# AHupuJR/REFID

Measured on AMD Instinct MI355X. Metric: interpolated frames/sec (train step) GoPro 256x256 11+1, higher is better.
Workload: dtype f32

## Files before the change

refid_amd/csrc/common.h:

```cpp
#pragma once
#include <hip/hip_runtime.h>
#include <stdint.h>
#include <stdio.h>
#include <stdarg.h>
#include <atomic>
#include "../../include/refid_hip.h"

typedef float f32x4 __attribute__((ext_vector_type(4)));
typedef float f32x16 __attribute__((ext_vector_type(16)));

void refid_set_error(const char* fmt, ...);

#define REFID_CHECK(cond, ...)                    \
    do {                                          \
        if (!(cond)) {                            \
            refid_set_error(__VA_ARGS__);         \
            return 1;                             \
        }                                         \
    } while (0)

#define REFID_LAUNCH_CHECK(what)                                                   \
    do {                                                                           \
        hipError_t e__ = hipGetLastError();                                        \
        if (e__ != hipSuccess) {                                                   \
// ... 8 lines not shown
#pragma unroll
        for (int k = 0; k < 4; ++k) v[k] = lrelu(v[k], slope);
        asm volatile("" ::: "memory");
    }
}

template <int LPP>
__device__ __forceinline__ float refid_wave_rows_sum(float v) {
#pragma unroll
    for (int o = LPP; o < 64; o <<= 1) v += __shfl_xor(v, o, 64);
    return v;
}

int refid_launch_sum_rows_f64(const double* part, int rows, int n, double* out, hipStream_t st);

static inline int cdiv(int a, int b) { return (a + b - 1) / b; }
static inline int round_up(int a, int b) { return cdiv(a, b) * b; }

template <class K>
static inline int refid_lds_attr_once(std::atomic<unsigned long long>& done, K kernel, int bytes, const char* what) {
    int dev = 0;
    if (hipGetDevice(&dev) != hipSuccess || dev < 0 || dev > 63) { refid_set_error("%s: hipGetDevice failed", what); return 2; }
    if ((done.load(std::memory_order_relaxed) >> dev) & 1ull) return 0;
    hipError_t e = hipFuncSetAttribute(reinterpret_cast<const void*>(kernel), hipFuncAttributeMaxDynamicSharedMemorySize, bytes);
    if (e != hipSuccess) { refid_set_error("%s: LDS attribute: %s", what, hipGetErrorString(e)); return 2; }
    done.fetch_or(1ull << dev, std::memory_order_relaxed);
    return 0;
}
```

refid_amd/csrc/conv_args.h:

```cpp
#pragma once

struct ConvKArgs {
    const float* inA; const float* inB;
    int ldA, ldB, Ca, Ctot;
    const float* w; const float* bias;
    float* out; int ldO;
    const float* res; int ldR;
    const float* mask; int ldM;
    int N, H, W, Ho, Wo;
    int Cout, CoutPad, coBase;
    int pad, nchunks, tilesX, tilesY;
    float slopePre, slopePost, slopeMask;
    long long wClsStride;
    int vecOK;
    int ncot;
    int bf16;
    int ksplit = 1;
    long long wsStride = 0;
    int gridTiles = 0;
    const float* add2 = nullptr; float* out2 = nullptr; int ldA2 = 0, ldO2 = 0;
    int maskMode = 0;
    int shuffle = 0;
    int patchW = 0, patchRow = 0;
};


size_t refid_wino3x3_workspace_bytes(const ConvKArgs& a, int split_mode);
int refid_launch_wino3x3(const ConvKArgs& a, float* ws, size_t ws_bytes, int split_mode, int tile_hint, hipStream_t st);
int refid_launch_splitk_finish(const ConvKArgs& f, const float* ws, int ldW, long long npix, hipStream_t st);
bool refid_wino6_eligible(const ConvKArgs& a);
size_t refid_wino6_workspace_bytes(const ConvKArgs& a, int split_mode);
int refid_launch_wino6(const ConvKArgs& a, float* ws, size_t ws_bytes, int split_mode, int tile_hint, int terms, hipStream_t st);
bool refid_split3x3_eligible(const ConvKArgs& a);
int refid_launch_split3x3(const ConvKArgs& a, int terms, int mode, int cus, int split_mode, hipStream_t st);
struct PwExtra {
    const float* lnG = nullptr; const float* lnB = nullptr; float lnEps = 0.f; float* lnOut = nullptr; int ldLn = 0;
    const float* pool = nullptr; int poolParts = 0; float invHW = 0.f; int hw = 0; int seC = 0;
    const float* seW1 = nullptr; const float* seB1 = nullptr; const float* seW2 = nullptr; const float* seB2 = nullptr;
// ... 7 lines not shown
```

refid_amd/csrc/conv_split.hip:

```cpp
#include "common.h"
#include "conv_args.h"

#ifndef REFID_SPLIT_ABLATE
#define REFID_SPLIT_ABLATE 0
#endif

namespace {

typedef __bf16 bf16x8 __attribute__((ext_vector_type(8)));
typedef _Float16 f16x8 __attribute__((ext_vector_type(8)));
typedef _Float16 f16x2 __attribute__((ext_vector_type(2)));
typedef float f32x2 __attribute__((ext_vector_type(2)));
constexpr int F16_TGT = 8;
constexpr int F16_SLACK = 6;
constexpr int F16_E0 = F16_TGT + 1;
constexpr int F16_HEADER = 64;
constexpr int TW = 32;
constexpr int KC = 8;
constexpr int NTH = 256;
constexpr int OOB = -1;
__device__ __forceinline__ int cdiv_dev(int a, int b) { return (a + b - 1) / b; }

#ifdef REFID_SPLIT_TRACE
__device__ unsigned long long* g_split_trace = nullptr;
// ... 57 lines not shown
__device__ __forceinline__ void split8h(const f32x4& v0, const f32x4& v1, f32x4 (&pl)[2]) {
    f16x8 h, l;
#pragma unroll
    for (int k = 0; k < 8; k += 2) {
        const f32x2 ab = {k < 4 ? v0[k] : v1[k - 4], k < 4 ? v0[k + 1] : v1[k - 3]};
        const f16x2 hh = __builtin_convertvector(ab, f16x2);
        const f32x2 r = ab - __builtin_convertvector(hh, f32x2);
        const f16x2 ll = __builtin_convertvector(r, f16x2);
        h[k] = hh[0]; h[k + 1] = hh[1];
        l[k] = ll[0]; l[k + 1] = ll[1];
    }
    pl[0] = __builtin_bit_cast(f32x4, h);
    pl[1] = __builtin_bit_cast(f32x4, l);
}

template <int MT, int NT, int PL, int KS, int MODE, bool F16 = false>
__global__ __launch_bounds__(NTH, 2) void conv_split_kernel(const ConvKArgs a) {
    using C = SCfg<MT, NT, PL, KS, MODE, F16>;
    static_assert(!F16 || PL == 2, "the fp16 form has two planes");
    constexpr int HP = C::HP, BN = C::BN, HWD = C::HWD, NTAP = C::NTAP, NSTEP = C::NSTEP;
    static_assert(MODE != 1 || KS == 2, "MODE 1: a stage = the two column positions of a block");
    extern __shared__ __attribute__((aligned(16))) char smem[];
    f32x4* sA = reinterpret_cast<f32x4*>(smem);
    f32x4* sB = sA + KS * PL * C::A_SLOTS;
    float* sM = reinterpret_cast<float*>(sB + KS * PL * C::B_SLOTS);

    const int tid = threadIdx.x;
    const int lane = tid & 63, wave = tid >> 6;
    const int li = lane & 31, kh = lane >> 5;

    const int xcd = blockIdx.x & 7, slot = blockIdx.x >> 3;
// ... 81 lines not shown
                    if constexpr (MODE == 1) vo = sub == 0 ? (sy1 ? voB[it] : voA[it]) : (sy1 ? vo1x[1][it] : vo1x[0][it]);
                    else vo = fromA ? voA[it] : voB[it];
                    if (!cok) vo = OOB;
                    ra[sub][it][i & 1] = __builtin_bit_cast(f32x4, __builtin_amdgcn_raw_buffer_load_b128(rs, vo, soff + 16 * (i & 1), 0));
                } else {
                    const int it = i - 2 * C::A_ITEMS;
                    int vo = voW[it];
                    if constexpr (MODE == 2) vo |= (ch * KS + sub < nsub) ? 0 : OOB;
                    rb[sub][it] = __builtin_bit_cast(
                        f32x4, __builtin_amdgcn_raw_buffer_load_b128(rsW, vo, (ch * KS + sub) * wChunk, 0));
                }
            }
        }
    };
    auto load_chunk = [&](int ch) { load_part(ch, -1); };
    auto post_max = [&]() {
        float tm = 0.f;
#pragma unroll
        for (int sub = 0; sub < KS; ++sub)
#pragma unroll
            for (int it = 0; it < C::A_ITEMS; ++it)
#pragma unroll
                for (int h = 0; h < 2; ++h) {
                    const f32x4 v = ra[sub][it][h];
                    tm = fmaxf(fmaxf(tm, fmaxf(fabsf(v[0]), fabsf(v[1]))), fmaxf(fabsf(v[2]), fabsf(v[3])));
                }
#pragma unroll
        for (int o = 32; o >= 1; o >>= 1) tm = fmaxf(tm, __shfl_xor(tm, o));
        if (lane == 0) sM[wave] = tm;
    };
// ... 60 lines not shown
            const int dy = (j == 0) ? 1 : (py ? 2 : 0);
            const int dx = (kh == 0) ? 1 : (px ? 2 : 0);
            aoff[j] = (wave * MT + dy) * HWD + dx + li;
        }
    }
    const f32x4* pB = sB + kh * BN + li;

    load_chunk(0);
    if constexpr (F16) {
        post_max();
        __syncthreads();
        store_chunk(stage_scale());
    } else {
        store_chunk();
    }
    __syncthreads();
    SPLIT_STAMP(1);

    for (int ch = 0; ch < ((REFID_SPLIT_ABLATE == 5 || REFID_SPLIT_ABLATE == 7) ? 0 : a.nchunks); ++ch) {
        const bool more = ch + 1 < a.nchunks;
        SPLIT_KSTAMP(ch, 0);
        SPLIT_KSTAMP(ch, 1);
#pragma unroll
        for (int sj = 0; sj < NSTEP * KS; ++sj) {
            const int sub = sj / NSTEP, j = sj % NSTEP;
            if (more && REFID_SPLIT_ABLATE != 4) load_part(ch + 1, sj);
            f32x4 af[PL][MT], bf[PL][NT];
#pragma unroll
            for (int p = 0; p < PL; ++p) {
#pragma unroll
                for (int m = 0; m < MT; ++m)
                    af[p][m] = REFID_SPLIT_ABLATE == 8 ? ra[0][0][m & 1] : sA[(sub * PL + p) * C::A_SLOTS + m * HWD + aoff[j]];
#pragma unroll
                for (int nn = 0; nn < NT; ++nn)
// ... 2 lines not shown
#pragma unroll
            for (int e = 0; e < (REFID_SPLIT_ABLATE == 1 ? 0 : TERMS); ++e)
#pragma unroll
                for (int m = 0; m < MT; ++m)
#pragma unroll
                    for (int nn = 0; nn < NT; ++nn) {
                        if constexpr (F16)
                            acc[m][nn] = __builtin_amdgcn_mfma_f32_32x32x16_f16(
                                __builtin_bit_cast(f16x8, bf[TB[e]][nn]), __builtin_bit_cast(f16x8, af[TA[e]][m]),
                                acc[m][nn], 0, 0, 0);
                        else
                            acc[m][nn] = __builtin_amdgcn_mfma_f32_32x32x16_bf16(
                                __builtin_bit_cast(bf16x8, bf[TB[e]][nn]), __builtin_bit_cast(bf16x8, af[TA[e]][m]),
                                acc[m][nn], 0, 0, 0);
                    }
            __builtin_amdgcn_sched_barrier(0);
        }
        SPLIT_KSTAMP(ch, 2);
        if constexpr (F16) {
            if (more) post_max();
        }
        __syncthreads();
        SPLIT_KSTAMP(ch, 3);
#ifdef REFID_SPLIT_TRACE
        __builtin_amdgcn_s_waitcnt(0x0F70);
#endif
        SPLIT_KSTAMP(ch, 4);
        if (more) {
            if constexpr (F16) store_chunk(stage_scale());
            else store_chunk();
            SPLIT_KSTAMP(ch, 5);
            __syncthreads();
        }
        SPLIT_KSTAMP(ch, 6);
    }
    SPLIT_STAMP(2);

    constexpr int C4 = C::C4, XS = C::XS;
    constexpr int EIT = (32 * C4) / 64;
    auto opix = [&](int oy, int ox) -> long long {
        if (MODE == 2) return (long long)(n * 2 * a.Ho + 2 * oy + py) * (2 * a.Wo) + 2 * ox + px;
        return (long long)(n * a.Ho + oy) * a.Wo + ox;
    };
    f32x4* ex = reinterpret_cast<f32x4*>(smem) + wave * (32 * XS);
#pragma unroll
    for (int m = 0; m < MT; ++m) {
        const int oy = oy0 + wave * MT + m;
        f32x4 pres[EIT], pmask[EIT];
        const bool pre = a.vecOK && (a.res != nullptr || a.mask != nullptr) && REFID_SPLIT_ABLATE != 6 && REFID_SPLIT_ABLATE != 7;
// ... 60 lines not shown
                for (int k = 0; k < 4; ++k) {
                    if (j0 + k >= a.Cout) break;
                    float tv = v[k];
                    if (a.res) tv += a.res[op * a.ldR + j0 + k];
                    tv = lrelu(tv, a.slopePost);
                    if (a.mask) tv *= (a.mask[op * a.ldM + j0 + k] > 0.f) ? 1.f : a.slopeMask;
                    a.out[op * a.ldO + j0 + k] = tv;
                    if (a.out2) a.out2[op * a.ldO2 + j0 + k] = tv + a.add2[op * a.ldA2 + j0 + k];
                }
            }
        }
    }
    SPLIT_STAMP(3);
}

template <int MT, int NT, int PL, int KS, int MODE, bool F16 = false>
int launch_split(const ConvKArgs& ka, hipStream_t st) {
    using C = SCfg<MT, NT, PL, KS, MODE, F16>;
    static std::atomic<unsigned long long> attr_done{0};
    if (int rc = refid_lds_attr_once(attr_done, &conv_split_kernel<MT, NT, PL, KS, MODE, F16>, C::LDS_BYTES, "conv_split")) return rc;
    ConvKArgs a = ka;
    a.tilesX = cdiv(a.Wo, TW);
    a.tilesY = cdiv(a.Ho, C::TH);
    a.nchunks = (MODE == 1) ? 2 * cdiv(a.Ctot, KC) : cdiv(a.Ctot, KC * KS);
    a.ncot = cdiv(a.Cout, C::BN);
    const int tiles = a.tilesX * a.tilesY * a.N;
    dim3 grid(cdiv(tiles, 8) * 8 * a.ncot, MODE == 2 ? 4 : 1);
    hipLaunchKernelGGL((conv_split_kernel<MT, NT, PL, KS, MODE, F16>), grid, dim3(NTH), C::LDS_BYTES, st, a);
    REFID_LAUNCH_CHECK("conv_split");
    return 0;
}

template <int PL, int MODE, bool F16 = false>
int launch_split_pl(const ConvKArgs& a, bool wide, bool tall, hipStream_t st) {
    constexpr int KS = (MODE == 0) ? 1 : 2;
    if (wide) return tall ? launch_split<2, 2, PL, KS, MODE, F16>(a, st) : launch_split<1, 2, PL, KS, MODE, F16>(a, st);
    return tall ? launch_split<2, 1, PL, KS, MODE, F16>(a, st) : launch_split<1, 1, PL, KS, MODE, F16>(a, st);
}

}

#ifdef REFID_SPLIT_TRACE
extern "C" int refid_split_trace_set(unsigned long long* wg_stamps, unsigned long long* k_stamps, int wg) {
    if (hipMemcpyToSymbol(HIP_SYMBOL(g_split_trace), &wg_stamps, sizeof(wg_stamps)) != hipSuccess) return 1;
    if (hipMemcpyToSymbol(HIP_SYMBOL(g_split_ktrace), &k_stamps, sizeof(k_stamps)) != hipSuccess) return 1;
// ... 38 lines not shown
```

refid_amd/csrc/conv_wino6.hip:

```cpp
#include "common.h"
#include "conv_args.h"
#include <algorithm>
#include <cstdlib>

#ifndef REFID_WINO6_ABLATE
#define REFID_WINO6_ABLATE 0
#endif

namespace {

constexpr int TW = 32;
constexpr int KC = 16;
constexpr int HWD = TW + 2;
constexpr int TH = 4;
constexpr int ROWP = 40;
constexpr int PLANE = 6 * ROWP + 5;
constexpr int R_F4 = 4 * PLANE;
constexpr int HP = (TH + 2) * HWD;
constexpr int R_ITEMS = (4 * HP + 255) / 256;
constexpr int lds_bytes(int nt) { return nt == 2 ? 64 * 66 * 16 : (32 * 66 * 16 > 2 * R_F4 * 16 ? 32 * 66 * 16 : 2 * R_F4 * 16); }
constexpr int OOB = -1;
typedef __bf16 bf16x8 __attribute__((ext_vector_type(8)));
typedef _Float16 f16x8 __attribute__((ext_vector_type(8)));
typedef _Float16 f16x2 __attribute__((ext_vector_type(2)));
// ... 34 lines not shown
    pl[0] = __builtin_bit_cast(f32x4, h);
    pl[1] = __builtin_bit_cast(f32x4, l);
}

__device__ __forceinline__ void round8h(const f32x4& v0, const f32x4& v1, f32x4 (&pl)[3]) {
    f16x8 h;
#pragma unroll
    for (int k = 0; k < 8; k += 2) {
        const f32x2 ab = {k < 4 ? v0[k] : v1[k - 4], k < 4 ? v0[k + 1] : v1[k - 3]};
        const f16x2 hh = __builtin_convertvector(ab, f16x2);
        h[k] = hh[0]; h[k + 1] = hh[1];
    }
    pl[0] = __builtin_bit_cast(f32x4, h);
}

template <int NT, bool F16, bool ONE = false>
__global__ __launch_bounds__(256, NT == 2 ? 2 : 3) void conv_wino6_kernel(const ConvKArgs a) {
    constexpr int BN = 32 * NT;
    static_assert(F16 || !ONE, "the one-product form is an fp16 form");
    constexpr int NPL = ONE ? 1 : (F16 ? 2 : 3);
    constexpr int NPR = ONE ? 1 : ((REFID_WINO6_ABLATE == 14 || REFID_WINO6_ABLATE == 15) ? 3 : (F16 ? 3 : 6));
    extern __shared__ __attribute__((aligned(16))) char smem[];
    f32x4* sR = reinterpret_cast<f32x4*>(smem);

    const int tid = threadIdx.x;
    const int lane = tid & 63, wave = tid >> 6;
    const int li = lane & 31, kh = lane >> 5;
    const int ti = wave;
    if (REFID_WINO6_ABLATE == 20 && a.N > 0) return;
    if (REFID_WINO6_ABLATE == 21 && a.N > 0) { __syncthreads(); if (tid == 12345) a.out[0] = 1.f; return; }

// ... 66 lines not shown
        for (int it = 0; it < R_ITEMS; ++it) sR[buf * R_F4 + sdst[it]] = src[it];
    };
    auto load_u = [&](int ch, int j, f32x4 (&dst)[NPL][NT]) {
        const bool in = ch < kc1;
        const int so = (REFID_WINO6_ABLATE == 1 ? 0 : ch) * uChunk + j * uXi;
#pragma unroll
        for (int p = 0; p < ((REFID_WINO6_ABLATE == 14 || REFID_WINO6_ABLATE == 15) && !ONE ? 2 : NPL); ++p)
#pragma unroll
            for (int nt = 0; nt < NT; ++nt) {
                if (REFID_WINO6_ABLATE == 13 && nt == 1) { dst[p][nt] = dst[p][0]; continue; }
                dst[p][nt] = __builtin_bit_cast(
                    f32x4, __builtin_amdgcn_raw_buffer_load_b128(rsW, in ? voU[nt] : OOB, in ? so + p * uPlane : 0, 0));
            }
    };

    f32x16 acc[4][NT];
#pragma unroll
    for (int j = 0; j < 4; ++j)
#pragma unroll
        for (int t = 0; t < NT; ++t)
#pragma unroll
            for (int r = 0; r < 16; ++r) acc[j][t][r] = 0.f;

    const int rowP = (ti == 0) ? 0 : ((ti == 2) ? 2 : 1);
    const int rowM = (ti == 0) ? 2 : ((ti == 1) ? 2 : ((ti == 2) ? 1 : 3));
    const float sgn = (ti == 1) ? 1.f : -1.f;
    const int tbase = 2 * kh * PLANE + (2 * (li >> 4)) * ROWP + (li & 15);
    const int offP = tbase + rowP * ROWP, offM = tbase + rowM * ROWP;
    constexpr int BOFF[4] = {0, 20, 1, 21};

    constexpr int TA[6] = {0, 0, 1, 0, 2, 1};
    constexpr int TB[6] = {0, 1, 0, 2, 0, 1};

    f32x4 uA[NPL][NT], uB[NPL][NT];
    auto phase = [&](int ch) {
        const int lc = ch - kc0;
        if (REFID_WINO6_ABLATE != 7 && REFID_WINO6_ABLATE != 8) {
            store_raw((lc + 1) & 1, rr);
            load_raw(ch + 2, rr);
#ifdef REFID_WINO6_PIN
            __builtin_amdgcn_sched_barrier(0x38F);
#endif
        }
        const f32x4* r = sR + (lc & 1) * R_F4;
        f32x4 t[2][4];
#pragma unroll
        for (int qq = 0; qq < 2; ++qq)
#pragma unroll
            for (int b = 0; b < 4; ++b) t[qq][b] = r[qq * PLANE + offP + BOFF[b]] + r[qq * PLANE + offM + BOFF[b]] * sgn;
        if constexpr (F16 && REFID_WINO6_ABLATE != 16) {
// ... 43 lines not shown
            else if (F16 && REFID_WINO6_ABLATE == 18) { pl[0] = v[0]; pl[1] = v[1]; }
            else if constexpr (ONE) round8h(v[0], v[1], pl);
            else if constexpr (F16) split8h(v[0], v[1], pl);
            else split8(v[0], v[1], pl);
#pragma unroll
            for (int e = 0; e < NPR; ++e)
#pragma unroll
                for (int nt = 0; nt < NT; ++nt) {
                    if constexpr (F16)
                        acc[j][nt] = __builtin_amdgcn_mfma_f32_32x32x16_f16(
                            __builtin_bit_cast(f16x8, cur[TB[e]][nt]), __builtin_bit_cast(f16x8, pl[TA[e]]), acc[j][nt], 0, 0, 0);
                    else
                        acc[j][nt] = __builtin_amdgcn_mfma_f32_32x32x16_bf16(
                            __builtin_bit_cast(bf16x8, cur[TB[e]][nt]), __builtin_bit_cast(bf16x8, pl[TA[e]]), acc[j][nt], 0, 0, 0);
                }
        }
        __syncthreads();
    };

    {
        f32x4 rr0[R_ITEMS];
#if REFID_WINO6_ABLATE == 19
        int keep[R_ITEMS];
#pragma unroll
        for (int it = 0; it < R_ITEMS; ++it) {
            keep[it] = pixo[it];
            const int hp = (tid >> 2) + it * 64;
            const int row = hp / HWD, col = hp % HWD;
            pixo[it] = (hp < HP && row >= a.pad && col >= a.pad) ? (row - a.pad) * a.W + (col - a.pad) : OOB;
        }
#endif
        load_raw(kc0, rr0);
        load_raw(kc0 + 1, rr);
#if REFID_WINO6_ABLATE == 19
#pragma unroll
        for (int it = 0; it < R_ITEMS; ++it) pixo[it] = keep[it];
#endif
        load_u(kc0, 0, uA);
        if (REFID_WINO6_ABLATE == 6 || REFID_WINO6_ABLATE == 8) load_u(kc0, 1, uB);
        store_raw(0, rr0);
    }
    __syncthreads();

    if (REFID_WINO6_ABLATE != 3 && REFID_WINO6_ABLATE != 10)
        for (int ch = kc0; ch < kc1; ++ch) phase(ch);

    constexpr int XL = 66;
    f32x4* xch = reinterpret_cast<f32x4*>(smem);
#pragma unroll
    for (int t = 0; t < NT; ++t)
#pragma unroll
        for (int rq = 0; rq < 4; ++rq) {
            f32x4 r0, r1;
#pragma unroll
            for (int k = 0; k < 4; ++k) {
                const int r = 4 * rq + k;
                r0[k] = acc[0][t][r] + acc[1][t][r] + acc[2][t][r];
                r1[k] = acc[1][t][r] - acc[2][t][r] - acc[3][t][r];
                if constexpr (F16) {
                    r0[k] = ldexpf(r0[k], eRef - 127 - F16_TGT - eU);
// ... 111 lines not shown
    a.nchunks = cdiv(a.Ctot, KC);
    a.ncot = cdiv(a.Cout, bn);
    p.grid = dim3(round_up(a.tilesX * a.tilesY * a.N, 8) * a.ncot);
    const int nwg = (split_mode == 2) ? (int)p.grid.x : a.tilesX * a.tilesY * a.ncot * 8;
    int ks = 1;
    if (split_mode && nwg <= 256 && a.nchunks >= 8) {
        ks = 512 / nwg;
        if (ks > a.nchunks / 4) ks = a.nchunks / 4;
        if (ks > 8) ks = 8;
        if (ks < 1) ks = 1;
    }
    p.ks = ks;
    return p;
}

template <int NT, bool F16, bool ONE = false>
int launch_wino6_t(const ConvKArgs& a, dim3 grid, hipStream_t st, const char* what) {
    static std::atomic<unsigned long long> done{0};
    if (int rc = refid_lds_attr_once(done, &conv_wino6_kernel<NT, F16, ONE>, lds_bytes(NT), "conv_wino6")) return rc;
    hipLaunchKernelGGL((conv_wino6_kernel<NT, F16, ONE>), grid, dim3(256), lds_bytes(NT), st, a);
    REFID_LAUNCH_CHECK(what);
    return 0;
}

template <int NT>
int launch_wino6(const ConvKArgs& a, int terms, dim3 grid, hipStream_t st, const char* what) {
    if (terms == 1) return launch_wino6_t<NT, true, true>(a, grid, st, what);
    return terms == 3 ? launch_wino6_t<NT, true>(a, grid, st, what) : launch_wino6_t<NT, false>(a, grid, st, what);
}

}

bool refid_wino6_eligible(const ConvKArgs& a) {
    const long long lim = 0x7fffffffLL;
    return a.Cout >= 1 && a.Ctot % 4 == 0 && (a.inB == nullptr || a.Ca % KC == 0) &&
           (long long)a.N * a.H * a.W * a.ldA * 4 < lim && (!a.inB || (long long)a.N * a.H * a.W * a.ldB * 4 < lim) &&
           (long long)cdiv(a.Ctot, KC) * 16 * 3 * a.CoutPad * KC * 2 < lim;
// ... 7 lines not shown
        if (p.ks > 1) need = std::max(need, (size_t)p.ks * a.N * a.Ho * a.Wo * round_up(a.Cout, 4) * sizeof(float));
    }
    return need;
}

int refid_launch_wino6(const ConvKArgs& ka, float* ws, size_t ws_bytes, int split_mode, int tile_hint, int terms, hipStream_t st) {
    ConvKArgs a = ka;
    REFID_CHECK(terms == 0 || terms == 6 || terms == 3 || terms == 1, "conv2d: algo 5 takes mfma_terms 0 / 6 (six bf16 products), 3 "
                "(three fp16 products, w_packed from refid_pack_conv_weights_wino3h) or 1 (one fp16 product, w_packed from "
                "refid_pack_conv_weights_wino1h), got %d", terms);
    const bool f16 = terms == 3 || terms == 1;
    REFID_CHECK(!f16 || (reinterpret_cast<uintptr_t>(a.w) & 15) == 0, "conv2d: the fp16 Winograd packing must be 16-byte aligned");
    REFID_CHECK(refid_wino6_eligible(a),
                "conv2d: the Winograd six-product tile needs input-channel counts that are multiples "
                "of 4 (two sources: c_a a multiple of 16) and tensors below 2 GiB");
    const Wino6Plan pl = wino6_plan(a, ws ? split_mode : 0, tile_hint);
    dim3 grid = pl.grid;
    const int ks = pl.ks;
    if (ks == 1) return pl.nt == 2 ? launch_wino6<2>(a, terms, grid, st, "conv_wino6") : launch_wino6<1>(a, terms, grid, st, "conv_wino6/32");
    const long long npix = (long long)a.N * a.Ho * a.Wo;
    const int ldW = round_up(a.Cout, 4);
    const size_t need = (size_t)ks * npix * ldW * sizeof(float);
    if (need > ws_bytes || (reinterpret_cast<uintptr_t>(ws) & 15)) {
        refid_set_error("conv_wino6: split-K workspace too small or misaligned (%zu bytes given, %zu needed: "
                        "refid_conv_workspace_bytes)", ws_bytes, need);
        return 1;
    }
    ConvKArgs p = a;
    p.ksplit = ks; p.wsStride = npix * ldW; p.out = ws; p.ldO = ldW; p.out2 = nullptr;
    grid.y = ks;
// ... 7 lines not shown
```

refid_amd/csrc/runtime.hip:

```cpp
#include "common.h"
#include <cstring>

static thread_local char g_err[512] = "";

void refid_set_error(const char* fmt, ...) {
    va_list ap;
    va_start(ap, fmt);
    vsnprintf(g_err, sizeof(g_err), fmt, ap);
    va_end(ap);
}

extern "C" const char* refid_last_error(void) { return g_err; }
extern "C" int refid_abi_version(void) { return REFID_ABI_VERSION; }
extern "C" int refid_experimental_tiles(void) {
    return 0;
}

extern "C" int refid_device_cu_count(void) {
    int dev = 0;
    if (hipGetDevice(&dev) != hipSuccess) return -1;
    hipDeviceProp_t p;
    if (hipGetDeviceProperties(&p, dev) != hipSuccess) return -1;
    return p.multiProcessorCount;
}
// ... 873 lines not shown
```

refid_amd/csrc/wgrad_wino24.hip:

```cpp
#include "common.h"
#include "wgrad_args.h"
#include <cstdlib>
#include <cstring>
#include <type_traits>
#include <vector>

#ifndef REFID_W24_ABLATE
#define REFID_W24_ABLATE 0
#endif
#define W24_NO_DMA (REFID_W24_ABLATE == 1 || REFID_W24_ABLATE == 5 || REFID_W24_ABLATE == 6)
#define W24_NO_MFMA (REFID_W24_ABLATE == 2)
#define W24_NO_LDS (REFID_W24_ABLATE == 3 || REFID_W24_ABLATE == 6)
#define W24_NO_BAR (REFID_W24_ABLATE == 4 || REFID_W24_ABLATE == 5 || REFID_W24_ABLATE == 6)

namespace {

__device__ __forceinline__ float w24_fake(float seed) { asm volatile("" : "+v"(seed)); return seed; }

constexpr int IT = 32;
constexpr int TC = 4;
constexpr int GH = 4, GW = 4 * TC;
constexpr int XH = GH + 2, XW = GW + 2;
constexpr int X_BYTES = XH * XW * IT * 4;
constexpr int GS_BYTES = GH * GW * 32 * 4;
constexpr int buf_bytes(int ns) { return X_BYTES + ns * GS_BYTES; }
constexpr int lds24_bytes(int ns) { return 2 * buf_bytes(ns); }
constexpr int NXI = 24;
typedef __attribute__((address_space(3))) void* lds_ptr24;
typedef __attribute__((address_space(3))) const float lds_cf24;
typedef float f32x2 __attribute__((ext_vector_type(2)));

template <int AH, int BH>
__device__ __forceinline__ f32x2 w24_pair(f32x2 a, f32x2 b) {
    f32x2 d;
    if constexpr (AH == 0 && BH == 0) asm("v_pk_mov_b32 %0, %1, %2 op_sel:[0,0]" : "=v"(d) : "v"(a), "v"(b));
    else if constexpr (AH == 1 && BH == 0) asm("v_pk_mov_b32 %0, %1, %2 op_sel:[1,0]" : "=v"(d) : "v"(a), "v"(b));
    else if constexpr (AH == 0 && BH == 1) asm("v_pk_mov_b32 %0, %1, %2 op_sel:[0,1]" : "=v"(d) : "v"(a), "v"(b));
    else asm("v_pk_mov_b32 %0, %1, %2 op_sel:[1,1]" : "=v"(d) : "v"(a), "v"(b));
    return d;
}

// ... 50 lines not shown
    static __device__ __forceinline__ void v_cols(const f32x2 (&t)[6], f32x2 (&v)[6]) {
        v[0] = 4.f * t[0] + (-5.f * t[2] + t[4]);
        v[1] = (t[3] + t[4]) - 4.f * (t[1] + t[2]);
        v[2] = 4.f * (t[1] - t[2]) + (t[4] - t[3]);
        const f32x2 d42 = t[4] - t[2], d31 = t[3] - t[1];
        v[3] = 2.f * d31 + d42;
        v[4] = d42 - 2.f * d31;
        v[5] = 4.f * t[1] + (-5.f * t[3] + t[5]);
    }
    static __device__ __forceinline__ void z_cols(const f32x2 (&x)[4], f32x2 (&z)[6]) {
        const f32x2 e = x[0] + x[2], o = x[1] + x[3], e4 = 4.f * x[2] + x[0], o4 = 4.f * x[3] + x[1];
        z[0] = x[0]; z[1] = e + o; z[2] = e - o; z[3] = 2.f * o4 + e4; z[4] = e4 - 2.f * o4; z[5] = x[3];
    }
};

template <int NS, bool DOWN>
__global__ __launch_bounds__(256, NS == 2 ? 2 : 3) void wgrad_wino24_kernel(const W24Args a) {
    constexpr int OT = 32 * NS, BUF_BYTES = buf_bytes(NS), XPS = DOWN ? 2 : 1;
    extern __shared__ __attribute__((aligned(16))) char smem[];
    const int tid = threadIdx.x, lane = tid & 63;
    const int wave = __builtin_amdgcn_readfirstlane(tid >> 6);
    const int li = lane & 31, kh = lane >> 5;
    const int phase = DOWN ? blockIdx.z / a.ncoT : 0, php = phase >> 1, phq = phase & 1;
    const int co0 = (DOWN ? blockIdx.z % a.ncoT : blockIdx.z) * OT, ci0 = blockIdx.y * IT;
    const int split = blockIdx.x;
    const int Hin = DOWN ? a.Hin : a.H, Win = DOWN ? a.Win : a.W;

    const bool xFromA = ci0 < a.Ca || ci0 >= a.Ctot;
    const int xld = xFromA ? a.ldA : a.ldB;
    const long long gpixAll = (long long)a.N * a.Ho * a.Wo, xpixAll = (long long)a.N * Hin * Win;
    const int limG = (int)min(gpixAll * a.ldG * 4, 0x7fffffffLL), limX = (int)min(xpixAll * xld * 4, 0x7fffffffLL);
// ... 1 lines not shown
    const int chunk = (ntAll + a.nsplit - 1) / a.nsplit;
    const int p0 = min(split * chunk, ntAll), p1 = min(p0 + chunk, ntAll);

    int qg, qn, qy, qx;
    {
        int t = p0 < ntAll ? p0 : 0;
        qg = t / a.ntiles; t -= qg * a.ntiles;
        qx = t % a.tilesX; t /= a.tilesX;
        qy = t % a.tilesY; qn = t / a.tilesY;
    }
    const int xq = ci0 + (lane & 7) * 4, xt = ci0 + (lane & 31), gq = co0 + (lane & 7) * 4;
    const int xlc = ((lane >> 3) * XPS * xld + (xFromA ? xq : xq - a.Ca)) * 4;
    const int xlt = ((lane >> 5) * XPS * xld + (xFromA ? xt : xt - a.Ca)) * 4;
    const int glc = ((lane >> 3) * a.ldG + gq) * 4;
    const bool fullch = ci0 + IT <= a.Ctot && co0 + OT <= a.Co;
    constexpr int OOB = 0x7ff00000;
    const int xRowB = XPS * Win * xld * 4, gRowB = a.Wo * a.ldG * 4;
    auto x_origin = [&](int n, int ty, int tx) {
        return ((n * Hin + XPS * (ty * GH - a.pad) + php) * Win + XPS * (tx * GW - a.pad) + phq) * xld * 4;
    };
    const float* gPtr = a.g[qg];
    const float* xPtr = xFromA ? a.inA[qg] : a.inB[qg];
    int xTile = x_origin(qn, qy, qx);
    int gTile = ((qn * a.Ho + qy * GH) * a.Wo + qx * GW) * a.ldG * 4;
    auto request = [&](int buf) {
        const int oy0 = qy * GH, ox0 = qx * GW;
        const int iy0 = oy0 - a.pad, ix0 = ox0 - a.pad;
        const __amdgpu_buffer_rsrc_t rsG = __builtin_amdgcn_make_buffer_rsrc(const_cast<float*>(gPtr), 0, limG, 0x00020000);
        const __amdgpu_buffer_rsrc_t rsX = __builtin_amdgcn_make_buffer_rsrc(const_cast<float*>(xPtr), 0, limX, 0x00020000);
        char* xdst = smem + buf * BUF_BYTES;
        char* gdst = xdst + X_BYTES;
        const bool fast = fullch && ix0 >= 0 && ix0 + XW <= a.W && ox0 + GW <= a.Wo && xld * 8 * XPS * 4 < 0x100000 && a.ldG * 8 * 4 < 0x100000;
        const int q0 = NS == 2 ? (wave < 2 ? wave : 3 * wave - 4) : 2 * (wave - 2), nq = NS == 2 ? (wave < 2 ? 1 : 3) : (wave < 2 ? 0 : 2);
        if (fast) {
#pragma unroll
            for (int k = 0; k < 2; ++k) {
                const int r = wave + 4 * k;
                if (r < XH && !W24_NO_DMA) {
                    const int base = (unsigned)(iy0 + r) < (unsigned)a.H ? xTile + r * xRowB : OOB;
// ... 58 lines not shown
            qx = 0;
            qy += 1;
            if (qy == a.tilesY) {
                qy = 0;
                qn += 1;
                if (qn == a.N) {
                    qn = 0;
                    qg = min(qg + 1, a.groups - 1);
                    gPtr = a.g[qg];
                    xPtr = xFromA ? a.inA[qg] : a.inB[qg];
                }
            }
            xTile = x_origin(qn, qy, 0);
            gTile = (qn * a.Ho + qy * GH) * a.Wo * a.ldG * 4;
        }
    };

    f32x16 acc[6][NS];
#pragma unroll
    for (int j = 0; j < 6; ++j)
#pragma unroll
        for (int sm = 0; sm < NS; ++sm)
#pragma unroll
            for (int r = 0; r < 16; ++r) acc[j][sm][r] = 0.f;
    float bs[NS];
#pragma unroll
    for (int sm = 0; sm < NS; ++sm) bs[sm] = 0.f;

    static_assert(BUF_BYTES % 256 == 0 && (BUF_BYTES + X_BYTES + (NS - 1) * GS_BYTES + 4 * GW * 32 * 4) / 256 < 256, "ds_read2st64 offset range");
    lds_cf24* xe = (lds_cf24*)smem + (2 * kh) * (XW * IT) + li;
// ... 30 lines not shown
                    f32x2 x[4], z[6];
                    R::g_rows(gbb, s, sm, x);
                    R::z_cols(x, z);
                    if constexpr (I == 1) bs[sm] += z[1][0] + z[1][1];
#pragma unroll
                    for (int h = 0; h < 2; ++h)
#pragma unroll
                        for (int j = 0; j < 6; ++j) {
                            if (W24_NO_MFMA) { asm volatile("" :: "v"(v[j][h]), "v"(z[j][h])); continue; }
                            acc[j][sm] = __builtin_amdgcn_mfma_f32_32x32x2f32(v[j][h], z[j][h], acc[j][sm], 0, 0, 0);
                        }
                }
            }
        };
        auto sync = [&] {
            __builtin_amdgcn_s_waitcnt(0x0F70);
            if (!W24_NO_BAR) __builtin_amdgcn_s_barrier();
            __builtin_amdgcn_sched_barrier(0);
        };
        const int npairs = (p1 - p0) >> 1;
        if (p0 < p1) request(0);
        for (int i = 0; i < npairs; ++i) {
            sync();
            request(1);
            tile(std::integral_constant<int, 0>{});
            sync();
            if (p0 + 2 * i + 2 < p1) request(0);
            tile(std::integral_constant<int, 1>{});
        }
        if ((p1 - p0) & 1) {
            sync();
            tile(std::integral_constant<int, 0>{});
        }
    };
    switch (wave) {
        case 0: kloop(std::integral_constant<int, 0>{}); break;
        case 1: kloop(std::integral_constant<int, 1>{}); break;
        case 2: kloop(std::integral_constant<int, 2>{}); break;
        default: kloop(std::integral_constant<int, 3>{}); break;
    }

#pragma unroll
    for (int j = 0; j < 6; ++j) {
        float* sl = a.slabs + ((long long)((split * (DOWN ? 4 : 1) + phase) * NXI + wave * 6 + j) * a.CoP) * a.CiP;
#pragma unroll
        for (int sm = 0; sm < NS; ++sm) {
            const int co = co0 + sm * 32 + li;
#pragma unroll
            for (int qd = 0; qd < 4; ++qd) {
                const int ci = ci0 + 8 * qd + 4 * kh;
                f32x4 vv;
#pragma unroll
                for (int k = 0; k < 4; ++k) vv[k] = acc[j][sm][4 * qd + k];
                f32x4* dst = reinterpret_cast<f32x4*>(sl + (long long)co * a.CiP + ci);
                if (a.accum) vv += *dst;
// ... 166 lines not shown
__global__ __launch_bounds__(256) void wgrad_wino24_reduce_down_kernel(const W24rArgs a) { w24_reduce_down_body(a, blockIdx.x); }

struct W24rBatch { W24rArgs job[REFID_FINISH_BATCH]; int blk0[REFID_FINISH_BATCH + 1]; int n; };
static_assert(sizeof(W24rBatch) <= 4096, "kernel-argument block");
__global__ __launch_bounds__(256) void wgrad_wino24_reduce_batch_kernel(const W24rBatch b) {
    __shared__ float part[256 * (NXI + 1)];
    int j = 0;
    for (int k = 1; k < b.n; ++k) j = (int)blockIdx.x >= b.blk0[k] ? k : j;
    const int blk = (int)blockIdx.x - b.blk0[j];
    if (b.job[j].down) w24_reduce_down_body(b.job[j], blk);
    else w24_reduce_body(b.job[j], blk, part);
}

struct W24rQueued { W24rArgs r; int nblocks; };
thread_local std::vector<W24rQueued> w24_queue;

struct Geo24 { int ncoT, nciT, tilesX, tilesY, ntiles, nsplit, CoP, CiP; };

int ns_of(const refid_wgrad_desc* d) { return d->c_o <= 32 ? 1 : 2; }
bool is_down(const refid_wgrad_desc* d) { return d->kh == 4; }

Geo24 geo24_of(const refid_wgrad_desc* d) {
    Geo24 g;
    const int OT = 32 * ns_of(d);
    g.ncoT = cdiv(d->c_o, OT);
    const int ci_geo = (d->phase != 0) ? d->i_total - d->i_base : d->c_a + d->c_b;
    g.nciT = cdiv(ci_geo > d->c_a + d->c_b ? ci_geo : d->c_a + d->c_b, IT);
    g.tilesX = cdiv(d->wo, GW);
    g.tilesY = cdiv(d->ho, GH);
    g.ntiles = g.tilesX * g.tilesY * d->n;
// ... 71 lines not shown
    w24_queue.clear();
    return 0;
}

namespace {
long long slab_floats(const refid_wgrad_desc* d, const Geo24& g) { return (long long)(is_down(d) ? 4 : 1) * NXI * g.CoP * g.CiP; }
}

size_t refid_wgrad_wino24_workspace_bytes(const refid_wgrad_desc* d) {
    const Geo24 g = geo24_of(d);
    const long long slab = slab_floats(d, g);
    return ((size_t)g.nsplit * slab + (size_t)g.nsplit * g.CoP + (size_t)refid_slab_fold_count(slab, g.nsplit) * slab) * sizeof(float);
}

int refid_wgrad_wino24_launch(const refid_wgrad_desc* d, hipStream_t st) {
    static std::atomic<unsigned long long> attr_done{0}, attr_done1{0}, attr_done2{0}, attr_done3{0};
    if (int rc = refid_lds_attr_once(attr_done, &wgrad_wino24_kernel<2, false>, lds24_bytes(2), "wgrad_wino24")) return rc;
    if (int rc = refid_lds_attr_once(attr_done1, &wgrad_wino24_kernel<1, false>, lds24_bytes(1), "wgrad_wino24<1>")) return rc;
    if (int rc = refid_lds_attr_once(attr_done2, &wgrad_wino24_kernel<2, true>, lds24_bytes(2), "wgrad_wino24<down>")) return rc;
    if (int rc = refid_lds_attr_once(attr_done3, &wgrad_wino24_kernel<1, true>, lds24_bytes(1), "wgrad_wino24<1, down>")) return rc;
    const Geo24 g = geo24_of(d);
    const bool down = is_down(d);
    const long long slab = slab_floats(d, g);
    if (down)
        REFID_CHECK(d->kw == 4 && d->stride == 2 && d->pad == 1 && d->h % 2 == 0 && d->w % 2 == 0 && d->ho == d->h / 2 && d->wo == d->w / 2,
                    "wgrad (algo 7): a 4x4 stride-2 pad-1 conv over an even-sized input");
    REFID_CHECK(d->c_b == 0 || d->c_a % IT == 0, "wgrad (Winograd 2x4 tiles): c_a must be a multiple of %d for two sources", IT);
    REFID_CHECK(d->ld_g % 4 == 0 && d->ld_a % 4 == 0 && (d->c_b == 0 || d->ld_b % 4 == 0) && d->c_o % 4 == 0 &&
                    d->c_a % 4 == 0 && d->c_b % 4 == 0,
                "wgrad (Winograd 2x4 tiles): pitches and channel counts must be multiples of 4 floats (16-byte LDS-DMA pieces)");
    {
        const long long lim = 0x7fffffffLL;
        REFID_CHECK((long long)d->n * d->ho * d->wo * d->ld_g * 4 < lim && (long long)d->n * d->h * d->w * d->ld_a * 4 < lim &&
                        (d->c_b == 0 || (long long)d->n * d->h * d->w * d->ld_b * 4 < lim),
                    "wgrad (Winograd 2x4 tiles): tensor too large for 32-bit buffer offsets (use algo 0)");
// ... 11 lines not shown
                    "wgrad (Winograd 2x4 tiles): tensors must be 16-byte aligned (group %d)", k);
    }
    a.groups = ngrp;
    a.ldG = d->ld_g; a.Co = d->c_o;
    a.ldA = d->ld_a; a.ldB = d->ld_b;
    a.Ca = d->c_a; a.Ctot = d->c_a + d->c_b;
    a.slabs = d->slabs;
    a.bslabs = d->db ? d->slabs + (size_t)g.nsplit * slab : nullptr;
    a.N = d->n; a.H = d->h; a.W = d->w; a.Ho = d->ho; a.Wo = d->wo; a.pad = d->pad;
    a.Hin = d->h; a.Win = d->w; a.ncoT = g.ncoT;
    if (down) { a.H = d->ho; a.W = d->wo; a.pad = 1; }
    a.tilesX = g.tilesX; a.tilesY = g.tilesY; a.ntiles = g.ntiles; a.nsplit = g.nsplit;
    a.CoP = g.CoP; a.CiP = g.CiP;
    a.accum = (d->phase == 2);
    if (d->phase != 3) {
        if (down) {
            if (ns_of(d) == 1)
                hipLaunchKernelGGL((wgrad_wino24_kernel<1, true>), dim3(g.nsplit, g.nciT, 4 * g.ncoT), dim3(256), lds24_bytes(1), st, a);
            else
                hipLaunchKernelGGL((wgrad_wino24_kernel<2, true>), dim3(g.nsplit, g.nciT, 4 * g.ncoT), dim3(256), lds24_bytes(2), st, a);
        } else if (ns_of(d) == 1)
            hipLaunchKernelGGL((wgrad_wino24_kernel<1, false>), dim3(g.nsplit, g.nciT, g.ncoT), dim3(256), lds24_bytes(1), st, a);
        else
            hipLaunchKernelGGL((wgrad_wino24_kernel<2, false>), dim3(g.nsplit, g.nciT, g.ncoT), dim3(256), lds24_bytes(2), st, a);
        REFID_LAUNCH_CHECK("wgrad_wino24");
    }
    if (d->phase == 1 || d->phase == 2) return 0;
    W24rArgs r;
    r.slabs = a.slabs; r.bslabs = a.bslabs; r.dw = d->dw; r.db = d->db;
    r.nsplit = g.nsplit; r.Co = d->o_real;
    int nred = g.nsplit;
    if (const int S = refid_slab_fold_count(slab, g.nsplit)) {
        const long long slabFloats = slab;
        float* part = d->slabs + (size_t)g.nsplit * slab + (size_t)g.nsplit * g.CoP;
        if (int rc = refid_launch_slab_fold(a.slabs, part, slabFloats, g.nsplit, S, st)) return rc;
        r.slabs = part;
        nred = S;
    }
    r.Ci = (d->phase == 0 && a.Ctot < d->i_total - d->i_base) ? a.Ctot : d->i_total - d->i_base;
// ... 27 lines not shown
```

Baseline: 501.9.

## Add L2 prefetch touches ahead of input loads in conv and wgrad kernels

Adds software prefetch "touch" loads that pull upcoming input cache lines into L2 ahead of their real use. The split-conv kernel touches two stages ahead, the Winograd-6 kernel touches up to three future channel chunks, and the wgrad Winograd 2x4 kernel issues an LDS-DMA touch of the next tile into a small dump area. It is on by default and can be switched off per kernel through an environment mask. The touches are meant to hide global-memory latency. In exchange they cost extra load instructions, registers, LDS and waitcnt stalls, and the conv-split kernel gains a ping-pong unrolled stage loop.

```diff
diff --git a/refid_amd/csrc/common.h b/refid_amd/csrc/common.h
--- a/refid_amd/csrc/common.h
+++ b/refid_amd/csrc/common.h
@@ -46,6 +46,10 @@
 
 int refid_launch_sum_rows_f64(const double* part, int rows, int n, double* out, hipStream_t st);
 
+constexpr int REFID_TOUCH_WINO6 = 1, REFID_TOUCH_SPLIT = 2, REFID_TOUCH_W24 = 4;
+constexpr int REFID_L2_TOUCH_DEFAULT = REFID_TOUCH_WINO6 | REFID_TOUCH_SPLIT | REFID_TOUCH_W24;
+int refid_l2_touch();
+
 static inline int cdiv(int a, int b) { return (a + b - 1) / b; }
 static inline int round_up(int a, int b) { return cdiv(a, b) * b; }
 
diff --git a/refid_amd/csrc/conv_args.h b/refid_amd/csrc/conv_args.h
--- a/refid_amd/csrc/conv_args.h
+++ b/refid_amd/csrc/conv_args.h
@@ -22,6 +22,7 @@
     int maskMode = 0;
     int shuffle = 0;
     int patchW = 0, patchRow = 0;
+    int touch = 0;
 };
 
 
diff --git a/refid_amd/csrc/conv_split.hip b/refid_amd/csrc/conv_split.hip
--- a/refid_amd/csrc/conv_split.hip
+++ b/refid_amd/csrc/conv_split.hip
@@ -1,5 +1,6 @@
 #include "common.h"
 #include "conv_args.h"
+#include <type_traits>
 
 #ifndef REFID_SPLIT_ABLATE
 #define REFID_SPLIT_ABLATE 0
@@ -95,7 +96,7 @@
     pl[1] = __builtin_bit_cast(f32x4, l);
 }
 
-template <int MT, int NT, int PL, int KS, int MODE, bool F16 = false>
+template <int MT, int NT, int PL, int KS, int MODE, bool F16 = false, bool TOUCH = false>
 __global__ __launch_bounds__(NTH, 2) void conv_split_kernel(const ConvKArgs a) {
     using C = SCfg<MT, NT, PL, KS, MODE, F16>;
     static_assert(!F16 || PL == 2, "the fp16 form has two planes");
@@ -207,6 +208,27 @@
         }
     };
     auto load_chunk = [&](int ch) { load_part(ch, -1); };
+    constexpr int NTCH = C::A_ITEMS * (MODE == 1 ? 2 : 1);
+    int tch[2][NTCH];
+#pragma unroll
+    for (int i = 0; i < NTCH; ++i) tch[1][i] = 0;
+    auto touch_stage = [&](int st, int (&dst)[NTCH]) {
+        const int c0 = (MODE == 1 ? (st >> 1) : st * KS) * KC;
+        const bool fromA = MODE != 0 || c0 < a.Ca;
+        const int soff = (fromA ? c0 : c0 - a.Ca) * 4;
+        const bool opens = soff % 128 == 0 || (fromA ? a.ldA : a.ldB) % 32 != 0;
+        const bool in = st < a.nchunks && c0 < a.Ctot && opens;
+        const bool sy1 = MODE == 1 && (st & 1);
+        const __amdgpu_buffer_rsrc_t rs = __builtin_amdgcn_make_buffer_rsrc(
+            const_cast<float*>(fromA ? a.inA : a.inB), 0, fromA ? limA : limB, 0x00020000);
+#pragma unroll
+        for (int i = 0; i < NTCH; ++i) {
+            int vo;
+            if constexpr (MODE == 1) vo = (i & 1) == 0 ? (sy1 ? voB[i >> 1] : voA[i >> 1]) : (sy1 ? vo1x[1][i >> 1] : vo1x[0][i >> 1]);
+            else vo = fromA ? voA[i] : voB[i];
+            dst[i] = __builtin_amdgcn_raw_buffer_load_b32(rs, vo | (in ? 0 : OOB), in ? soff : 0, 0);
+        }
+    };
     auto post_max = [&]() {
         float tm = 0.f;
 #pragma unroll
@@ -297,10 +319,12 @@
     } else {
         store_chunk();
     }
+    if constexpr (TOUCH) __builtin_amdgcn_s_waitcnt(0x0F70);
     __syncthreads();
     SPLIT_STAMP(1);
 
-    for (int ch = 0; ch < ((REFID_SPLIT_ABLATE == 5 || REFID_SPLIT_ABLATE == 7) ? 0 : a.nchunks); ++ch) {
+    auto stage = [&](int ch, auto PAR) {
+        constexpr int TP = decltype(PAR)::value;
         const bool more = ch + 1 < a.nchunks;
         SPLIT_KSTAMP(ch, 0);
         SPLIT_KSTAMP(ch, 1);
@@ -333,6 +357,7 @@
                                 __builtin_bit_cast(bf16x8, bf[TB[e]][nn]), __builtin_bit_cast(bf16x8, af[TA[e]][m]),
                                 acc[m][nn], 0, 0, 0);
                     }
+            if (TOUCH && sj == NSTEP * KS - 1 && REFID_SPLIT_ABLATE == 0) touch_stage(ch + 2, tch[TP]);
             __builtin_amdgcn_sched_barrier(0);
         }
         SPLIT_KSTAMP(ch, 2);
@@ -349,9 +374,28 @@
             if constexpr (F16) store_chunk(stage_scale());
             else store_chunk();
             SPLIT_KSTAMP(ch, 5);
+            if constexpr (TOUCH) {
+                __builtin_amdgcn_s_waitcnt(0x0F70 | (NTCH & 15));
+#pragma unroll
+                for (int i = 0; i < NTCH; ++i) asm volatile("" :: "v"(tch[TP ^ 1][i]));
+            }
             __syncthreads();
         }
         SPLIT_KSTAMP(ch, 6);
+    };
+    {
+        const int nst = (REFID_SPLIT_ABLATE == 5 || REFID_SPLIT_ABLATE == 7) ? 0 : a.nchunks;
+        if constexpr (TOUCH) {
+            int ch = 0;
+            for (; ch + 1 < nst; ch += 2) {
+                stage(ch, std::integral_constant<int, 0>{});
+                stage(ch + 1, std::integral_constant<int, 1>{});
+            }
+            if (ch < nst) stage(ch, std::integral_constant<int, 0>{});
+        } else {
+            for (int ch = 0; ch < ((REFID_SPLIT_ABLATE == 5 || REFID_SPLIT_ABLATE == 7) ? 0 : a.nchunks); ++ch)
+                stage(ch, std::integral_constant<int, 0>{});
+        }
     }
     SPLIT_STAMP(2);
 
@@ -442,11 +486,11 @@
     SPLIT_STAMP(3);
 }
 
-template <int MT, int NT, int PL, int KS, int MODE, bool F16 = false>
-int launch_split(const ConvKArgs& ka, hipStream_t st) {
+template <int MT, int NT, int PL, int KS, int MODE, bool F16, bool TOUCH>
+int launch_split_t(const ConvKArgs& ka, hipStream_t st) {
     using C = SCfg<MT, NT, PL, KS, MODE, F16>;
     static std::atomic<unsigned long long> attr_done{0};
-    if (int rc = refid_lds_attr_once(attr_done, &conv_split_kernel<MT, NT, PL, KS, MODE, F16>, C::LDS_BYTES, "conv_split")) return rc;
+    if (int rc = refid_lds_attr_once(attr_done, &conv_split_kernel<MT, NT, PL, KS, MODE, F16, TOUCH>, C::LDS_BYTES, "conv_split")) return rc;
     ConvKArgs a = ka;
     a.tilesX = cdiv(a.Wo, TW);
     a.tilesY = cdiv(a.Ho, C::TH);
@@ -454,9 +498,14 @@
     a.ncot = cdiv(a.Cout, C::BN);
     const int tiles = a.tilesX * a.tilesY * a.N;
     dim3 grid(cdiv(tiles, 8) * 8 * a.ncot, MODE == 2 ? 4 : 1);
-    hipLaunchKernelGGL((conv_split_kernel<MT, NT, PL, KS, MODE, F16>), grid, dim3(NTH), C::LDS_BYTES, st, a);
+    hipLaunchKernelGGL((conv_split_kernel<MT, NT, PL, KS, MODE, F16, TOUCH>), grid, dim3(NTH), C::LDS_BYTES, st, a);
     REFID_LAUNCH_CHECK("conv_split");
     return 0;
+}
+template <int MT, int NT, int PL, int KS, int MODE, bool F16 = false>
+int launch_split(const ConvKArgs& a, hipStream_t st) {
+    if (MODE != 0 && (refid_l2_touch() & REFID_TOUCH_SPLIT)) return launch_split_t<MT, NT, PL, KS, MODE, F16, MODE != 0>(a, st);
+    return launch_split_t<MT, NT, PL, KS, MODE, F16, false>(a, st);
 }
 
 template <int PL, int MODE, bool F16 = false>
diff --git a/refid_amd/csrc/conv_wino6.hip b/refid_amd/csrc/conv_wino6.hip
--- a/refid_amd/csrc/conv_wino6.hip
+++ b/refid_amd/csrc/conv_wino6.hip
@@ -2,6 +2,7 @@
 #include "conv_args.h"
 #include <algorithm>
 #include <cstdlib>
+#include <type_traits>
 
 #ifndef REFID_WINO6_ABLATE
 #define REFID_WINO6_ABLATE 0
@@ -72,7 +73,7 @@
     pl[0] = __builtin_bit_cast(f32x4, h);
 }
 
-template <int NT, bool F16, bool ONE = false>
+template <int NT, bool F16, bool ONE = false, bool TOUCH = false>
 __global__ __launch_bounds__(256, NT == 2 ? 2 : 3) void conv_wino6_kernel(const ConvKArgs a) {
     constexpr int BN = 32 * NT;
     static_assert(F16 || !ONE, "the one-product form is an fp16 form");
@@ -169,6 +170,27 @@
             }
     };
 
+    constexpr int MAXT = 3;
+    int tch[MAXT];
+    auto touch_raw = [&]() {
+        const int row = tid / HWD, col = tid % HWD;
+        const int iy = oy0 - a.pad + row, ix = ox0 - a.pad + col;
+        const int tpix = (tid < HP && iy >= 0 && iy < a.H && ix >= 0 && ix < a.W) ? (n * a.H + iy) * a.W + ix : OOB;
+        const bool pair = a.ldA % 32 == 0 && (!a.inB || (a.ldB % 32 == 0 && a.Ca % 32 == 0));
+        const int c1 = pair ? ((kc0 + 3) & ~1) : kc0 + 2;
+#pragma unroll
+        for (int i = 0; i < MAXT; ++i) {
+            const int ch = c1 + i * (pair ? 2 : 1);
+            const bool in = i < a.touch && ch < kc1;
+            const int c0 = in ? ch * KC : 0;
+            const bool fromA = c0 < a.Ca;
+            const __amdgpu_buffer_rsrc_t rs = __builtin_amdgcn_make_buffer_rsrc(
+                const_cast<float*>(fromA ? a.inA : a.inB), 0, fromA ? limA : limB, 0x00020000);
+            const int vo = (tpix * ((fromA ? a.ldA : a.ldB) * 4)) | (in ? 0 : OOB);
+            tch[i] = __builtin_amdgcn_raw_buffer_load_b32(rs, vo, (fromA ? c0 : c0 - a.Ca) * 4, 0);
+        }
+    };
+
     f32x16 acc[4][NT];
 #pragma unroll
     for (int j = 0; j < 4; ++j)
@@ -188,7 +210,7 @@
     constexpr int TB[6] = {0, 1, 0, 2, 0, 1};
 
     f32x4 uA[NPL][NT], uB[NPL][NT];
-    auto phase = [&](int ch) {
+    auto phase = [&](int ch, auto FIRST) {
         const int lc = ch - kc0;
         if (REFID_WINO6_ABLATE != 7 && REFID_WINO6_ABLATE != 8) {
             store_raw((lc + 1) & 1, rr);
@@ -262,6 +284,10 @@
                         acc[j][nt] = __builtin_amdgcn_mfma_f32_32x32x16_bf16(
                             __builtin_bit_cast(bf16x8, cur[TB[e]][nt]), __builtin_bit_cast(bf16x8, pl[TA[e]]), acc[j][nt], 0, 0, 0);
                 }
+            if (TOUCH && decltype(FIRST)::value && j == 0) {
+#pragma unroll
+                for (int i = 0; i < MAXT; ++i) asm volatile("" :: "v"(tch[i]));
+            }
         }
         __syncthreads();
     };
@@ -284,6 +310,7 @@
 #pragma unroll
         for (int it = 0; it < R_ITEMS; ++it) pixo[it] = keep[it];
 #endif
+        if constexpr (TOUCH) touch_raw();
         load_u(kc0, 0, uA);
         if (REFID_WINO6_ABLATE == 6 || REFID_WINO6_ABLATE == 8) load_u(kc0, 1, uB);
         store_raw(0, rr0);
@@ -291,7 +318,12 @@
     __syncthreads();
 
     if (REFID_WINO6_ABLATE != 3 && REFID_WINO6_ABLATE != 10)
-        for (int ch = kc0; ch < kc1; ++ch) phase(ch);
+    if constexpr (TOUCH) {
+        if (kc0 < kc1) phase(kc0, std::true_type{});
+        for (int ch = kc0 + 1; ch < kc1; ++ch) phase(ch, std::false_type{});
+    } else {
+        for (int ch = kc0; ch < kc1; ++ch) phase(ch, std::false_type{});
+    }
 
     constexpr int XL = 66;
     f32x4* xch = reinterpret_cast<f32x4*>(smem);
@@ -433,13 +465,17 @@
     return p;
 }
 
+template <int NT, bool F16, bool ONE, bool TOUCH>
+int launch_wino6_tt(const ConvKArgs& a, dim3 grid, hipStream_t st, const char* what) {
+    static std::atomic<unsigned long long> done{0};
+    if (int rc = refid_lds_attr_once(done, &conv_wino6_kernel<NT, F16, ONE, TOUCH>, lds_bytes(NT), "conv_wino6")) return rc;
+    hipLaunchKernelGGL((conv_wino6_kernel<NT, F16, ONE, TOUCH>), grid, dim3(256), lds_bytes(NT), st, a);
+    REFID_LAUNCH_CHECK(what);
+    return 0;
+}
 template <int NT, bool F16, bool ONE = false>
 int launch_wino6_t(const ConvKArgs& a, dim3 grid, hipStream_t st, const char* what) {
-    static std::atomic<unsigned long long> done{0};
-    if (int rc = refid_lds_attr_once(done, &conv_wino6_kernel<NT, F16, ONE>, lds_bytes(NT), "conv_wino6")) return rc;
-    hipLaunchKernelGGL((conv_wino6_kernel<NT, F16, ONE>), grid, dim3(256), lds_bytes(NT), st, a);
-    REFID_LAUNCH_CHECK(what);
-    return 0;
+    return a.touch ? launch_wino6_tt<NT, F16, ONE, true>(a, grid, st, what) : launch_wino6_tt<NT, F16, ONE, false>(a, grid, st, what);
 }
 
 template <int NT>
@@ -477,6 +513,8 @@
     REFID_CHECK(refid_wino6_eligible(a),
                 "conv2d: the Winograd six-product tile needs input-channel counts that are multiples "
                 "of 4 (two sources: c_a a multiple of 16) and tensors below 2 GiB");
+    static const int touch_lines = []() { const char* e = getenv("REFID_L2_TOUCH_LINES"); return e ? std::min(std::max(atoi(e), 0), 3) : 3; }();
+    a.touch = (refid_l2_touch() & REFID_TOUCH_WINO6) ? touch_lines : 0;
     const Wino6Plan pl = wino6_plan(a, ws ? split_mode : 0, tile_hint);
     dim3 grid = pl.grid;
     const int ks = pl.ks;
diff --git a/refid_amd/csrc/runtime.hip b/refid_amd/csrc/runtime.hip
--- a/refid_amd/csrc/runtime.hip
+++ b/refid_amd/csrc/runtime.hip
@@ -1,4 +1,5 @@
 #include "common.h"
+#include <cstdlib>
 #include <cstring>
 
 static thread_local char g_err[512] = "";
@@ -8,6 +9,11 @@
     va_start(ap, fmt);
     vsnprintf(g_err, sizeof(g_err), fmt, ap);
     va_end(ap);
+}
+
+int refid_l2_touch() {
+    static const int mask = []() { const char* e = getenv("REFID_L2_TOUCH"); return e ? atoi(e) : REFID_L2_TOUCH_DEFAULT; }();
+    return mask;
 }
 
 extern "C" const char* refid_last_error(void) { return g_err; }
diff --git a/refid_amd/csrc/wgrad_wino24.hip b/refid_amd/csrc/wgrad_wino24.hip
--- a/refid_amd/csrc/wgrad_wino24.hip
+++ b/refid_amd/csrc/wgrad_wino24.hip
@@ -24,7 +24,9 @@
 constexpr int X_BYTES = XH * XW * IT * 4;
 constexpr int GS_BYTES = GH * GW * 32 * 4;
 constexpr int buf_bytes(int ns) { return X_BYTES + ns * GS_BYTES; }
-constexpr int lds24_bytes(int ns) { return 2 * buf_bytes(ns); }
+constexpr int DUMP_BYTES = 4 * 256;
+constexpr int lds24_bytes(int ns) { return 2 * buf_bytes(ns) + DUMP_BYTES; }
+constexpr int NTOUCH = 1;
 constexpr int NXI = 24;
 typedef __attribute__((address_space(3))) void* lds_ptr24;
 typedef __attribute__((address_space(3))) const float lds_cf24;
@@ -105,7 +107,7 @@
     }
 };
 
-template <int NS, bool DOWN>
+template <int NS, bool DOWN, bool TOUCH>
 __global__ __launch_bounds__(256, NS == 2 ? 2 : 3) void wgrad_wino24_kernel(const W24Args a) {
     constexpr int OT = 32 * NS, BUF_BYTES = buf_bytes(NS), XPS = DOWN ? 2 : 1;
     extern __shared__ __attribute__((aligned(16))) char smem[];
@@ -137,8 +139,8 @@
     const int xlt = ((lane >> 5) * XPS * xld + (xFromA ? xt : xt - a.Ca)) * 4;
     const int glc = ((lane >> 3) * a.ldG + gq) * 4;
     const bool fullch = ci0 + IT <= a.Ctot && co0 + OT <= a.Co;
+    const int xRowB = XPS * Win * xld * 4, gRowB = a.Wo * a.ldG * 4;
     constexpr int OOB = 0x7ff00000;
-    const int xRowB = XPS * Win * xld * 4, gRowB = a.Wo * a.ldG * 4;
     auto x_origin = [&](int n, int ty, int tx) {
         return ((n * Hin + XPS * (ty * GH - a.pad) + php) * Win + XPS * (tx * GW - a.pad) + phq) * xld * 4;
     };
@@ -146,6 +148,12 @@
     const float* xPtr = xFromA ? a.inA[qg] : a.inB[qg];
     int xTile = x_origin(qn, qy, qx);
     int gTile = ((qn * a.Ho + qy * GH) * a.Wo + qx * GW) * a.ldG * 4;
+    constexpr int DEAD = (int)0x80000000;
+    const int tc = wave < 2 ? ((lane < 3 * XW && ci0 < a.Ctot)
+                                   ? (3 * wave + lane / XW) * xRowB + ((lane % XW) * XPS * xld + (xFromA ? ci0 : ci0 - a.Ca)) * 4 : DEAD)
+                            : ((((lane >> 4) & 1) < NS && co0 + ((lane >> 4) & 1) * 32 < a.Co)
+                                   ? (2 * (wave - 2) + (lane >> 5)) * gRowB + ((lane & 15) * a.ldG + co0 + ((lane >> 4) & 1) * 32) * 4 : DEAD);
+    int qi = 0;
     auto request = [&](int buf) {
         const int oy0 = qy * GH, ox0 = qx * GW;
         const int iy0 = oy0 - a.pad, ix0 = ox0 - a.pad;
@@ -234,6 +242,13 @@
             xTile = x_origin(qn, qy, 0);
             gTile = (qn * a.Ho + qy * GH) * a.Wo * a.ldG * 4;
         }
+        qi += 1;
+        if constexpr (TOUCH) {
+            const __amdgpu_buffer_rsrc_t ts = __builtin_amdgcn_make_buffer_rsrc(const_cast<float*>(wave < 2 ? xPtr : gPtr), 0,
+                                                                                wave < 2 ? limX : limG, 0x00020000);
+            const int base = p0 + qi < p1 ? (wave < 2 ? xTile : gTile) : DEAD;
+            __builtin_amdgcn_raw_ptr_buffer_load_lds(ts, (lds_ptr24)(smem + 2 * BUF_BYTES + wave * 256), 4, base + tc, 0, 0, 0);
+        }
     };
 
     f32x16 acc[6][NS];
@@ -294,7 +309,7 @@
             }
         };
         auto sync = [&] {
-            __builtin_amdgcn_s_waitcnt(0x0F70);
+            __builtin_amdgcn_s_waitcnt(TOUCH ? (0x0F70 | NTOUCH) : 0x0F70);
             if (!W24_NO_BAR) __builtin_amdgcn_s_barrier();
             __builtin_amdgcn_sched_barrier(0);
         };
@@ -319,6 +334,7 @@
         case 2: kloop(std::integral_constant<int, 2>{}); break;
         default: kloop(std::integral_constant<int, 3>{}); break;
     }
+    __builtin_amdgcn_s_waitcnt(0x0F70);
 
 #pragma unroll
     for (int j = 0; j < 6; ++j) {
@@ -515,6 +531,18 @@
 
 struct W24rQueued { W24rArgs r; int nblocks; };
 thread_local std::vector<W24rQueued> w24_queue;
+
+template <int NS, bool DOWN, bool TOUCH>
+int launch_w24_t(const W24Args& a, dim3 grid, hipStream_t st) {
+    static std::atomic<unsigned long long> attr_done{0};
+    if (int rc = refid_lds_attr_once(attr_done, &wgrad_wino24_kernel<NS, DOWN, TOUCH>, lds24_bytes(NS), "wgrad_wino24")) return rc;
+    hipLaunchKernelGGL((wgrad_wino24_kernel<NS, DOWN, TOUCH>), grid, dim3(256), lds24_bytes(NS), st, a);
+    return 0;
+}
+template <int NS, bool DOWN>
+int launch_w24(const W24Args& a, dim3 grid, bool touch, hipStream_t st) {
+    return touch ? launch_w24_t<NS, DOWN, true>(a, grid, st) : launch_w24_t<NS, DOWN, false>(a, grid, st);
+}
 
 struct Geo24 { int ncoT, nciT, tilesX, tilesY, ntiles, nsplit, CoP, CiP; };
 
@@ -616,11 +644,7 @@
 }
 
 int refid_wgrad_wino24_launch(const refid_wgrad_desc* d, hipStream_t st) {
-    static std::atomic<unsigned long long> attr_done{0}, attr_done1{0}, attr_done2{0}, attr_done3{0};
-    if (int rc = refid_lds_attr_once(attr_done, &wgrad_wino24_kernel<2, false>, lds24_bytes(2), "wgrad_wino24")) return rc;
-    if (int rc = refid_lds_attr_once(attr_done1, &wgrad_wino24_kernel<1, false>, lds24_bytes(1), "wgrad_wino24<1>")) return rc;
-    if (int rc = refid_lds_attr_once(attr_done2, &wgrad_wino24_kernel<2, true>, lds24_bytes(2), "wgrad_wino24<down>")) return rc;
-    if (int rc = refid_lds_attr_once(attr_done3, &wgrad_wino24_kernel<1, true>, lds24_bytes(1), "wgrad_wino24<1, down>")) return rc;
+    const bool touch = REFID_W24_ABLATE == 0 && (refid_l2_touch() & REFID_TOUCH_W24);
     const Geo24 g = geo24_of(d);
     const bool down = is_down(d);
     const long long slab = slab_floats(d, g);
@@ -662,15 +686,11 @@
     a.CoP = g.CoP; a.CiP = g.CiP;
     a.accum = (d->phase == 2);
     if (d->phase != 3) {
-        if (down) {
-            if (ns_of(d) == 1)
-                hipLaunchKernelGGL((wgrad_wino24_kernel<1, true>), dim3(g.nsplit, g.nciT, 4 * g.ncoT), dim3(256), lds24_bytes(1), st, a);
-            else
-                hipLaunchKernelGGL((wgrad_wino24_kernel<2, true>), dim3(g.nsplit, g.nciT, 4 * g.ncoT), dim3(256), lds24_bytes(2), st, a);
-        } else if (ns_of(d) == 1)
-            hipLaunchKernelGGL((wgrad_wino24_kernel<1, false>), dim3(g.nsplit, g.nciT, g.ncoT), dim3(256), lds24_bytes(1), st, a);
-        else
-            hipLaunchKernelGGL((wgrad_wino24_kernel<2, false>), dim3(g.nsplit, g.nciT, g.ncoT), dim3(256), lds24_bytes(2), st, a);
+        const dim3 grid(g.nsplit, g.nciT, (down ? 4 : 1) * g.ncoT);
+        int rc;
+        if (ns_of(d) == 1) rc = down ? launch_w24<1, true>(a, grid, touch, st) : launch_w24<1, false>(a, grid, touch, st);
+        else rc = down ? launch_w24<2, true>(a, grid, touch, st) : launch_w24<2, false>(a, grid, touch, st);
+        if (rc) return rc;
         REFID_LAUNCH_CHECK("wgrad_wino24");
     }
     if (d->phase == 1 || d->phase == 2) return 0;
```

New measurement: 496.9. 1.0% lower.
